# Abhipray/audio-codec

Hardware: AMD Instinct MI355X
Metric: audio channel-frames/s encode (48 kHz, 1024-line long blocks, 128 kb/s/ch) (higher is better)
Workload: dtype f64

## Files before the change

audio-codec_amd/csrc/k_psy.hip:

```cpp
#include "pacx_launch.h"
#include "mdct_dev.h"
#include "pcm_stage.h"
#include "wave_np_sum.h"
#include "quant_dev.h"


template <int DT>
__device__ __forceinline__ double hann_sample(const typename PcmStage<DT>::elem *raw, int i,
                                              const double *__restrict__ hw,
                                              const double *__restrict__ hw_pcm)
{
    if constexpr (DT == 0) {
        const int c = raw[i];
        return hw_pcm[i] * (double)(c == -32768 ? 0 : c);
    } else {
        return hw[i] * raw[i];
    }
}

#ifdef PACX_PSY_DEBUG
__device__ long long g_psy_dbg[16 * 16];
#define PSY_T(k) do { long long t_; asm volatile("s_waitcnt lgkmcnt(0)\n\ts_memtime %0\n\ts_waitcnt lgkmcnt(0)" : "=s"(t_) :: "memory"); \
                      if (dbg_on) dbg_acc[k] += t_ - dbg_last; dbg_last = t_; } while (0)
extern "C" int pacx_debug_read_psy(long long *out, int n)
// ... 591 lines not shown
#endif
#ifndef MASK_WG_PER_CU_PLAIN
#define MASK_WG_PER_CU_PLAIN 4
#endif



__device__ __forceinline__ unsigned long long mask_key_of(double v)
{
    const unsigned long long u = (unsigned long long)__double_as_longlong(v);
    return (u >> 63) ? ~u : (u | 0x8000000000000000ull);
}
__device__ __forceinline__ double mask_value_of(unsigned long long k)
{
    const unsigned long long u = (k >> 63) ? (k & 0x7fffffffffffffffull) : ~k;
    return __longlong_as_double((long long)u);
}

#ifndef MASK_WAVES_PLAIN
#define MASK_WAVES_PLAIN 4
#endif
constexpr int mask_waves(int m, bool tail) { return (m == PACX_M_LONG && !tail) ? MASK_WAVES_PLAIN : MASK_WAVES; }

template <int M, bool TAIL>
__global__ __launch_bounds__(64 * mask_waves(M, TAIL), (M == PACX_M_LONG && !TAIL) ? MASK_OCC_PLAIN : MASK_OCC) void k_mask(PacxTables T, const uint8_t *__restrict__ flags,
                                                         int n_ch, long long n_units, int mixed,
                                                         const PacxPeak *__restrict__ peaks,
                                                         const int32_t *__restrict__ n_peaks,
                                                         const double *__restrict__ lines,
                                                         double *__restrict__ smr,
                                                         double *__restrict__ thr_out,
                                                         const int32_t *__restrict__ cf_list,
                                                         const int32_t *__restrict__ cf_count,
                                                         MaskTail tail)
{
    constexpr bool SHORT = (M == PACX_M_SHORT);
    constexpr int NW = mask_waves(M, TAIL);
    static_assert(!(TAIL && SHORT), "the fused tail is for long blocks");
    constexpr int PER = M / 64;
    constexpr bool BARK_LDS = (MASK_LDS_TABLES & 1) != 0, QUIET_LDS = (MASK_LDS_TABLES & 2) != 0;
    __shared__ __attribute__((aligned(16))) double bark_l[BARK_LDS ? M : 1];
    __shared__ __attribute__((aligned(16))) double quiet_l[QUIET_LDS ? M : 1];
    __shared__ __attribute__((aligned(16))) double chunk_c[PER][4];
    constexpr bool PAD = M / 64 == 16;
    constexpr int RJ = PAD ? PER / 2 : 0;
    constexpr int NH = PAD ? 2 : 1, HP = PER / NH;
    constexpr int MH = M / NH;
    constexpr int JSTR = PAD ? 72 : 64;
    __shared__ __attribute__((aligned(16))) double bufs[NW][MH + (PAD ? MH / 8 : 0)];
    __shared__ __attribute__((aligned(16))) double2 mk_zs_all[NW][64];
    __shared__ __attribute__((aligned(16))) double mk_u_all[NW][64];
    const int tid = threadIdx.x, lane = tid & 63, wv = tid >> 6;
    const double *__restrict__ bark_g = SHORT ? T.bark_short : T.bark_long;
    const double *__restrict__ quiet_g = SHORT ? T.thresh_short : T.thresh_long;
    for (int i = tid; i < M; i += 64 * NW) {
        if (BARK_LDS)
            bark_l[i] = bark_g[i];
// ... 7 lines not shown
        double qm = quiet_s[64 * j + lane];
#pragma unroll
        for (int off = 32; off > 0; off >>= 1)
            qm = fmin(qm, __shfl_xor(qm, off, 64));
        if (lane == 0) {
            chunk_c[j][0] = bark_s[64 * j] - 0.5;
            chunk_c[j][1] = bark_s[64 * j + 63] + 0.5;
            chunk_c[j][2] = qm - 0.01;
        }
    }
    __syncthreads();

    double *buf = bufs[wv];
    const int sl = lane + (PAD ? lane >> 3 : 0);
    double2 *mk_zs = mk_zs_all[wv];
    double *mk_u = mk_u_all[wv];
    const int nb = SHORT ? T.nb_short : T.nb_long;
    const int32_t *__restrict__ lower = SHORT ? T.band_lower_short : T.band_lower_long;
    const int32_t *__restrict__ count = SHORT ? T.band_lines_short : T.band_lines_long;
    if (cf_list)
        n_units = SHORT ? (long long)(*cf_count) * PACX_SUB : (long long)(*cf_count);
#ifdef PACX_PSY_DEBUG
    const bool dbg_on = blockIdx.x == 5;
    long long dbg_acc[8] = {0, 0, 0, 0, 0, 0, 0, 0}, dbg_last = 0;
    unsigned long long st_pairs = 0, st_surv = 0, st_live = 0, st_batches = 0;
    PSY_T(7);
    dbg_acc[7] = 0;
#endif
    for (long long unit = (long long)blockIdx.x * NW + wv; unit < n_units;
         unit += (long long)gridDim.x * NW) {
        long long cf = SHORT ? unit / PACX_SUB : unit;
        const int sb = SHORT ? (int)(unit % PACX_SUB) : 0;
        if (cf_list) {
            cf = cf_list[cf];
        } else if (mixed) {
            const unsigned fl = flags ? flags[cf / n_ch] : 0u;
            if (SHORT != ((fl & 2u) != 0))
                continue;
        }
        const PacxPeak *__restrict__ pk = peaks + cf * PACX_MAX_PEAKS + sb * 64;
        const int np = n_peaks[cf * PACX_SUB + sb];
        const long long loff = cf * PACX_M_LONG + sb * PACX_M_SHORT;

        double rb[RJ ? RJ : 1];
#pragma unroll
        for (int j = 0; j < PER; ++j) {
            if (j < RJ)
// ... 73 lines not shown
                        pus[u] = mk_u[bs[u]];
                    }
#pragma unroll
                    for (int u = 0; u < 4; ++u) {
                        const double pz = zs[u].x, ps = zs[u].y, pu = pus[u];
                        const double dz = zj - pz;
                        const double a = fmax(fabs(dz) - 0.5, 0.0);
                        const double gain = (dz < 0.0 ? -27.0 : pu) * a;
                        const double cand = (ps + gain) - 16.0;
                        asm("v_max_f64 %0, %1, %2" : "=v"(bj) : "v"(bj), "v"(cand));
                    }
                }
                if (j < RJ)
                    rb[j] = bj;
                else
                    buf[sl + JSTR * (j - RJ)] = bj;
            }
        }
        wave_lds_fence();
        PSY_T(1);
        double *__restrict__ out = smr ? smr + cf * T.band_stride + sb * T.nb_short : nullptr;
        unsigned long long *key = (unsigned long long *)mk_zs;
        key[lane] = 0ull;
#pragma unroll 1
        for (int h = NH - 1; h >= 0; --h) {
            if (RJ && h == 0) {
                wave_lds_fence();
#pragma unroll
                for (int j = 0; j < RJ; ++j)
                    buf[sl + JSTR * j] = rb[j];
                wave_lds_fence();
            }
            const int k0 = h * MH;
            double v_next = lines[loff + k0 + lane], q_next = quiet_s[k0 + lane];
#pragma unroll 1
            for (int j = 0; j < HP; ++j) {
                const int k = k0 + lane + 64 * j;
                const double v = v_next;
                double thr = q_next;
                if (j + 1 < HP) {
                    v_next = lines[loff + k + 64];
                    q_next = quiet_s[k + 64];
                }
                const double bst = buf[sl + JSTR * j];
                if (bst > -INFINITY)
                    thr = fmax(thr, mask_round_trip(bst));
                if (thr_out)
                    thr_out[loff + k] = thr;
                double it = (v * v) * 4.0;
                if (it == 0.0)
                    it = 1e-8;
                double spl = 96.0 + 10.0 * pacx_log10_pos(it + PACX_EPS);
                if (spl < -30.0)
                    spl = -30.0;
                buf[sl + JSTR * j] = spl - thr;
            }
            wave_lds_fence();
            int rl = lane;
            asm volatile("" : "+v"(rl));
            double v[HP];
            uint8_t bd[HP];
            if constexpr (SHORT) {
                const double2 t = *(const double2 *)(buf + 2 * rl);
                v[0] = t.x;
                v[1] = t.y;
                const uchar2 b2 = *(const uchar2 *)(T.line_band_short + 2 * rl);
                bd[0] = b2.x;
                bd[1] = b2.y;
            } else {
                static_assert(SHORT || HP == 8, "eight lines per lane and half");
                const uint2 b8 = *(const uint2 *)(T.line_band_long + k0 + 8 * rl);
                const unsigned w[2] = {b8.x, b8.y};
#pragma unroll
                for (int j = 0; j < HP; ++j) {
                    v[j] = buf[9 * rl + j];
                    bd[j] = (uint8_t)(w[j >> 2] >> (8 * (j & 3)));
                }
            }
            wave_lds_fence();
            int cur = bd[0];
            double mx = v[0];
#pragma unroll
            for (int j = 1; j < HP; ++j) {
                if (bd[j] != cur) {
                    atomicMax(&key[cur], mask_key_of(mx));
                    cur = bd[j];
                    mx = v[j];
                } else {
                    mx = fmax(mx, v[j]);
                }
            }
            atomicMax(&key[cur], mask_key_of(mx));
        }
        wave_lds_fence();
        PSY_T(2);
        const double s_l = mask_value_of(key[lane & 31]);
        if (out && lane < nb)
            out[lane] = s_l;
        {
            if constexpr (TAIL) {
                wave_lds_fence();
                int tl = lane;
                asm volatile("" : "+v"(tl));
                char *base = (char *)buf;
                unsigned *words = (unsigned *)base;
                double *cp = (double *)(base + PACX_PAYLOAD_STRIDE);
                unsigned long long *bmax = (unsigned long long *)(base + 2704);
                int *ba_s = (int *)(base + 2960), *sf_s = ba_s + PACX_MAX_BANDS;
                int *offs = sf_s + PACX_MAX_BANDS, *lower_s = offs + PACX_MAX_BANDS + 1;
                const int half = tl >> 5, l = tl & 31;
                const unsigned fl = flags ? flags[cf / n_ch] : 0u;
                const long long boff = cf * T.band_stride;
                const int32_t *__restrict__ n_lines = T.use_sbr ? T.band_lines_long_alloc : T.band_lines_long;
                const double budget = pacx_bit_budget(T.target_bps, PACX_M_LONG, 0, (fl & 5u) != 0, T.n_scale_bits,
                                                      T.n_mant_size_bits, nb, T.use_vq, T.use_sbr);
// ... 72 lines not shown
                        if (tail.mantissa)
                            *(int4 *)(tail.mantissa + loff + k0 + j4) = make_int4(mq[0], mq[1], mq[2], mq[3]);
                    }
                    if (tail.status && __builtin_amdgcn_ballot_w64(near) && tl == 0)
                        atomicOr(&tail.status[cf], 16u);
                    if (tail.payload) {
                        wave_lds_fence();
                        const int nbytes = ((end - 3) + 4 + 7) >> 3;
                        unsigned *dst = (unsigned *)(tail.payload + cf * (long long)tail.payload_stride);
                        for (int i = tl; i < (nbytes + 3) / 4; i += 64)
                            dst[i] = __builtin_bswap32(words[i]);
                        if (tl == 0)
                            tail.n_bytes[cf] = nbytes;
                    }
                    PSY_T(6);
                }
            }
        }
        wave_lds_fence();
        PSY_T(3);
    }
#ifdef PACX_PSY_DEBUG
    if (dbg_on && lane == 0 && M == PACX_M_LONG)
        for (int k = 0; k < 8; ++k)
            g_psy_dbg[wv * 16 + k] = dbg_acc[k];
    if (lane == 0 && M == PACX_M_LONG) {
        atomicAdd((unsigned long long *)&g_psy_dbg[160], st_pairs);
        atomicAdd((unsigned long long *)&g_psy_dbg[161], st_surv);
        atomicAdd((unsigned long long *)&g_psy_dbg[162], st_live);
        atomicAdd((unsigned long long *)&g_psy_dbg[163], st_batches);
    }
#endif
}

#define SMRG_THREADS 256
__global__ __launch_bounds__(SMRG_THREADS) void k_smr_generic(long long n_blocks, int n, int nb,
                                                             const double *__restrict__ data,
                                                             const double *__restrict__ lines,
                                                             const double *__restrict__ hann,
                                                             const double *__restrict__ tw_cos,
                                                             const double *__restrict__ tw_sin, double norm,
                                                             double fstep, const double *__restrict__ bark,
                                                             const double *__restrict__ quiet,
                                                             const int32_t *__restrict__ band_lower,
                                                             const int32_t *__restrict__ band_count,
                                                             double *__restrict__ smr, double *__restrict__ thr_out,
                                                             int32_t *__restrict__ n_peaks_out)
{
    extern __shared__ __attribute__((aligned(16))) unsigned char smrg_lds[];
    const int half = n / 2, n_bins = half + 1, max_pk = half / 2 + 1;
    double *w = (double *)smrg_lds;
    double *inten = w + n;
    PacxPeak *pk = (PacxPeak *)(inten + n_bins + (n_bins & 1));
    __shared__ int n_pk;
    const int tid = threadIdx.x;
// ... 112 lines not shown
        launch_side<0, true>(T, in, flags, n_cf, short_blocks, mixed, peaks, n_peaks, n_kept, sbr_mean,
                             sbr_overall, st);
    else if (dtype == 0)
        launch_side<0, false>(T, in, flags, n_cf, short_blocks, mixed, peaks, n_peaks, n_kept, sbr_mean,
                              sbr_overall, st);
    else
        launch_side<1, false>(T, in, flags, n_cf, short_blocks, mixed, peaks, n_peaks, n_kept, sbr_mean,
                              sbr_overall, st);
}

void pacx_k::pacx_launch_front_long(const PacxTables &T, const PacxPcmView &in, long long n_cf, double *lines,
                                    int32_t *overall_scale, uint32_t *status, PacxPeak *peaks, int32_t *n_peaks,
                                    int32_t *n_kept, hipStream_t st)
{
    if (n_cf > 0)
        hipLaunchKernelGGL(k_front_long, dim3((unsigned)n_cf), dim3(64), 0, st, T, in, n_cf, lines, overall_scale,
                           status, peaks, n_peaks, n_kept);
}

void pacx_k::pacx_launch_mask(const PacxTables &T, const uint8_t *flags, int n_ch, long long n_cf,
                      int short_blocks, int mixed, const PacxPeak *peaks, const int32_t *n_peaks,
                      const double *lines, double *smr, double *thr_out, int n_cu,
                      const int32_t *list_long, const int32_t *list_short, const int32_t *counts,
                      const MaskTail *tail, hipStream_t st)
{
    if (n_cf <= 0)
        return;
    const int part = mixed >> 4;
    mixed &= 15;
    if ((!short_blocks || mixed) && part != 2) {
        const int nw = tail ? MASK_WAVES : MASK_WAVES_PLAIN;
        long long blocks = (n_cf + nw - 1) / nw;
        const long long per_cu = tail ? MASK_WG_PER_CU : MASK_WG_PER_CU_PLAIN;
        if (blocks > per_cu * n_cu)
            blocks = per_cu * n_cu;
        if (tail)
            hipLaunchKernelGGL((k_mask<PACX_M_LONG, true>), dim3((unsigned)blocks), dim3(64 * MASK_WAVES), 0, st, T,
                               flags, n_ch, n_cf, mixed, peaks, n_peaks, lines, (double *)nullptr, thr_out,
                               mixed ? list_long : nullptr, counts, *tail);
        else
            hipLaunchKernelGGL((k_mask<PACX_M_LONG, false>), dim3((unsigned)blocks), dim3(64 * MASK_WAVES_PLAIN), 0, st, T,
                               flags, n_ch, n_cf, mixed, peaks, n_peaks, lines, smr, thr_out,
                               mixed ? list_long : nullptr, counts, MaskTail{});
    }
    if ((short_blocks || mixed) && part != 1) {
        const long long units = n_cf * PACX_SUB;
        long long blocks = (units + MASK_WAVES - 1) / MASK_WAVES;
        if (blocks > (32LL / MASK_WAVES) * n_cu)
            blocks = (32LL / MASK_WAVES) * n_cu;
        hipLaunchKernelGGL((k_mask<PACX_M_SHORT, false>), dim3((unsigned)blocks), dim3(64 * MASK_WAVES), 0, st, T,
                           flags, n_ch, units, mixed, peaks, n_peaks, lines, smr, thr_out,
                           mixed ? list_short : nullptr, counts ? counts + 1 : nullptr, MaskTail{});
    }
}
```

audio-codec_amd/csrc/pacx_api.hip:

```cpp
#include <hip/hip_runtime.h>

#include <math.h>
#include <stdio.h>
#include <stdlib.h>
#include <string.h>

#include <cmath>
#include <string>
#include <vector>

#include "../../include/pacx.h"
#include "body_index.h"
#include "pacx_launch.h"
#include "pvq_dev.h"
#include "pacx_vq_tables.h"
#include "pacx_tables_gen.h"

using namespace pacx_k;

struct PacxOverrides {
    int split_short;
    int fuse_tail;
    int fuse_front;
    int vq_fuse_alloc;
    int vq_frame;
    int vq_bfs;
    int vq_dec_frame;
};

#define PACX_FUSE_FRONT_DEFAULT 1

static int env_override(const char *name, int lo, int hi)
{
    const char *e = getenv(name);
    if (!e || !*e)
        return -1;
    char *end;
    const long v = strtol(e, &end, 10);
    return (*end || v < lo || v > hi) ? -1 : (int)v;
}

static PacxOverrides read_overrides(void)
{
    PacxOverrides o;
    o.split_short = env_override("PACX_SPLIT_SHORT", 0, 0);
    o.fuse_tail = env_override("PACX_FUSE_TAIL", 0, 1);
    o.fuse_front = env_override("PACX_FUSE_FRONT", 0, 1);
    o.vq_fuse_alloc = env_override("PACX_VQ_FUSE_ALLOC", 0, 1);
    o.vq_frame = env_override("PACX_VQ_FRAME", 0, 0);
    o.vq_bfs = env_override("PACX_VQ_BFS", 0, 1 << 20);
    o.vq_dec_frame = env_override("PACX_VQ_DEC_FRAME", 0, 0);
    return o;
}

struct pacx_handle {
    int device;
    int n_cu;
    PacxOverrides force;
    PacxTables T;
    std::vector<void *> owned;
    long long ws_cf;
    double *ws_lines;
    double *ws_smr;
    PacxPeak *ws_peaks;
    int32_t *ws_npeaks;
    int32_t *ws_nkept;
    int32_t *ws_overall;
    long long *ws_chunks;
    long long *ws_offs;
    int32_t *ws_lists;
// ... 12 lines not shown
    int32_t *ws_mant;
    long long ws_dec_cf;
    double *ws_dec_lines;
    uint8_t *ws_dec_sbr;
    uint32_t *ws_dec_status;
    double *ws_sbr_mean;
    long long ws_vq_cf;
    unsigned *ws_unit_words;
    int32_t *ws_unit_bits;
    long long ws_index_bytes;
    char *ws_index;
    long long ws_thr_cf;
    double *ws_thr;
    uint32_t *ws_rate_status;
    long long ws_solve_n;
    char *ws_solve;
    long long *ws_seg;
    long long seg_host_n;
    long long *seg_host;
    hipEvent_t ev_seg;
    std::string err;
};

static thread_local std::string g_create_err;

static int fail(pacx_handle *h, int code, const std::string &msg)
{
    if (h)
        h->err = msg;
    else
        g_create_err = msg;
    return code;
}

#define HIP_TRY(h, call)                                                               \
    do {                                                                               \
        hipError_t e_ = (call);                                                        \
        if (e_ != hipSuccess)                                                          \
            return fail(h, PACX_E_HIP, std::string(#call) + ": " + hipGetErrorString(e_)); \
    } while (0)

static void drain_internal(pacx_handle *h);
#define HIP_TRY_FORKED(h, call)                                                        \
    do {                                                                               \
        hipError_t e_ = (call);                                                        \
        if (e_ != hipSuccess) {                                                        \
// ... 655 lines not shown
extern "C" int pacx_smr_batch(pacx_handle *h, const pacx_pcm *in, const double *lines, int short_blocks,
                              double *smr, double *threshold, int32_t *n_peaks, void *stream)
{
    if (!h)
        return PACX_E_ARG;
    PacxPcmView v;
    int fast;
    long long n_cf;
    int rc = check_pcm(h, in, &v, &fast, &n_cf);
    if (rc)
        return rc;
    if (n_cf == 0)
        return PACX_OK;
    if (!lines || !smr)
        return fail(h, PACX_E_ARG, "pacx_smr_batch: lines or smr is null");
    HIP_TRY(h, hipSetDevice(h->device));
    if ((rc = pacx_reserve(h, n_cf)))
        return rc;
    hipStream_t st = (hipStream_t)stream;
    const int sb = short_blocks ? 1 : 0;
    pacx_launch_side(h->T, v, in->dtype, fast, nullptr, n_cf, sb, 0, h->ws_peaks, h->ws_npeaks, h->ws_nkept,
                     nullptr, nullptr, st);
    pacx_launch_mask(h->T, nullptr, in->n_channels, n_cf, sb, 0, h->ws_peaks, h->ws_nkept, lines, smr,
                     threshold, h->n_cu, nullptr, nullptr, nullptr, nullptr, st);
    if (n_peaks) {
        if (sb)
            HIP_TRY(h, hipMemcpyAsync(n_peaks, h->ws_npeaks, (size_t)n_cf * PACX_SUB * sizeof(int32_t),
                                      hipMemcpyDeviceToDevice, st));
        else
            HIP_TRY(h, hipMemcpy2DAsync(n_peaks, sizeof(int32_t), h->ws_npeaks, PACX_SUB * sizeof(int32_t),
                                        sizeof(int32_t), (size_t)n_cf, hipMemcpyDeviceToDevice, st));
    }
    return post_launch(h, "pacx_smr_batch");
}

extern "C" int pacx_smr_generic_batch(pacx_handle *h, int64_t n_blocks, int n_samples, const double *data,
                                      const double *lines, const pacx_smr_tables *t, double *smr, double *threshold,
                                      int32_t *n_peaks, void *stream)
{
    if (!h)
        return PACX_E_ARG;
    if (n_blocks == 0)
        return PACX_OK;
    if (n_blocks < 0 || !data || !lines || !smr || !t || !t->hann || !t->tw_cos || !t->tw_sin || !t->bark ||
        !t->quiet || !t->band_lower || !t->band_lines)
        return fail(h, PACX_E_ARG, "pacx_smr_generic_batch: bad argument");
    if (n_samples < 16 || n_samples > 8192 || (n_samples & 1) || t->n_bands < 1 || t->n_bands > PACX_MAX_BANDS)
// ... 76 lines not shown
    {
        if (fast) {
            mdct_long(st);
            if (mixed)
                mdct_short(st);
        } else {
            pacx_launch_mdct(h->T, v, dtype, fast, frame_flags, n_cf, 0, mixed, 0, h->ws_lines, overall_scale, PACX_SUB,
                             status, st);
        }
    }
    void side(int part, bool sbr, hipStream_t st) const
    {
        pacx_launch_side(h->T, v, dtype, fast, frame_flags, n_cf, 0, mixed | part, h->ws_peaks, h->ws_npeaks, h->ws_nkept,
                         sbr ? h->ws_sbr_mean : nullptr, sbr ? overall_scale : nullptr, st);
    }
    void front_long(hipStream_t st) const
    {
        pacx_launch_front_long(h->T, v, n_cf, h->ws_lines, overall_scale, status, h->ws_peaks, h->ws_npeaks,
                               h->ws_nkept, st);
    }
    void mask(int part, const MaskTail *tail, hipStream_t st) const
    {
        pacx_launch_mask(h->T, frame_flags, n_ch, n_cf, 0, mixed | part, h->ws_peaks, h->ws_nkept, h->ws_lines, h->ws_smr,
                         nullptr, h->n_cu, list_long, list_short, counts, tail, st);
    }
};

static int encode_scalar(pacx_handle *h, const pacx_pcm *in, const uint8_t *frame_flags,
                         int32_t *overall_scale, int32_t *scale_factor, int32_t *bit_alloc,
                         int32_t *mantissa, uint32_t *status, uint8_t *payload, int32_t *n_bytes,
                         void *stream, const char *what)
{
    if (!h)
        return PACX_E_ARG;
    PacxPcmView v;
    int fast;
    long long n_cf;
    int rc = check_pcm(h, in, &v, &fast, &n_cf);
    if (rc)
        return rc;
    if (n_cf == 0)
        return PACX_OK;
    if (!overall_scale || !scale_factor || !bit_alloc || !status || (!payload && !mantissa) ||
        (payload && !n_bytes))
        return fail(h, PACX_E_ARG, std::string(what) + ": null output pointer");
    if (h->T.use_vq)
        return fail(h, PACX_E_UNSUPPORTED, std::string(what) + ": handle was created with use_vq "
// ... 580 lines not shown
{
    if (!h)
        return PACX_E_ARG;
    PacxPcmView v;
    int fast;
    long long n_cf;
    int rc = check_pcm(h, in, &v, &fast, &n_cf);
    if (rc)
        return rc;
    if (n_cf == 0)
        return PACX_OK;
    if (!dec_lines || !overall_scale || !noise || !mask || !nmr_db)
        return fail(h, PACX_E_ARG, "pacx_nmr_batch: null pointer");
    HIP_TRY(h, hipSetDevice(h->device));
    if ((rc = pacx_reserve(h, n_cf)) || (rc = grow(h, GROW_NMR, n_cf)))
        return rc;
    hipStream_t st = (hipStream_t)stream;
    const EncodeStep s(h, in, v, fast, frame_flags, n_cf, h->ws_overall, nullptr);
    if (s.mixed)
        s.lists(st);
    s.mdct(st);
    s.side(0, false, st);
    pacx_launch_mask(h->T, frame_flags, s.n_ch, n_cf, 0, s.mixed, h->ws_peaks, h->ws_nkept, h->ws_lines, h->ws_smr,
                     h->ws_thr, h->n_cu, s.list_long, s.list_short, s.counts, nullptr, st);
    pacx_launch_nmr(h->T, frame_flags, s.n_ch, n_cf, h->ws_lines, dec_lines, overall_scale, h->ws_thr, status, noise, mask,
                    nmr_db, st);
    return post_launch(h, "pacx_nmr_batch");
}

enum { BUDGET_SEARCH, BUDGET_GIVEN, ALLOC_GIVEN };
static int encode_budgeted(pacx_handle *h, const pacx_pcm *in, const uint8_t *frame_flags, int mode,
                           double target_nmr_db, double max_bits_per_sample, const int32_t *budget_in,
                           const int32_t *alloc_in, int32_t *overall_scale, int32_t *scale_factor, int32_t *bit_alloc, int32_t *mantissa,
                           uint32_t *status, uint8_t *payload, int32_t *n_bytes, int32_t *budget_out, void *stream,
                           const char *what)
{
    if (!h)
        return PACX_E_ARG;
    if (h->T.use_vq || h->T.use_sbr)
        return fail(h, PACX_E_UNSUPPORTED, std::string(what) + ": scalar handles only (created without use_vq, use_sbr)");
    const bool search = mode == BUDGET_SEARCH, given = mode == ALLOC_GIVEN;
    if (search && !std::isfinite(target_nmr_db))
        return fail(h, PACX_E_ARG, std::string(what) + ": target_nmr_db is not finite");
    if (search && !(max_bits_per_sample > 0.0 && max_bits_per_sample <= 16.0))
        return fail(h, PACX_E_ARG, std::string(what) + ": max_bits_per_sample must lie in (0, 16]");
    PacxPcmView v;
    int fast;
// ... 6 lines not shown
        return fail(h, PACX_E_ARG, std::string(what) + ": null pointer");
    if (n_cf == 0)
        return PACX_OK;
    HIP_TRY(h, hipSetDevice(h->device));
    if ((rc = pacx_reserve(h, n_cf)) || (search && (rc = grow(h, GROW_NMR, n_cf))))
        return rc;
    if (!mantissa) {
        if ((rc = grow(h, GROW_MANT, n_cf)))
            return rc;
        mantissa = h->ws_mant;
    }
    hipStream_t st = (hipStream_t)stream;
    if (!fast) {
        HIP_TRY(h, hipMemsetAsync(status, 0, (size_t)n_cf * sizeof(uint32_t), st));
        HIP_TRY(h, hipMemsetAsync(overall_scale, 0, (size_t)n_cf * PACX_SUB * sizeof(int32_t), st));
    }
    const EncodeStep s(h, in, v, fast, frame_flags, n_cf, overall_scale, status);
    if (s.mixed)
        s.lists(st);
    s.mdct(st);
    if (!given) {
        s.side(0, false, st);
        pacx_launch_mask(h->T, frame_flags, s.n_ch, n_cf, 0, s.mixed, h->ws_peaks, h->ws_nkept, h->ws_lines, h->ws_smr,
                         search ? h->ws_thr : nullptr, h->n_cu, s.list_long, s.list_short, s.counts, nullptr, st);
    }
    if (given)
        pacx_launch_band_sanitize(h->T, frame_flags, s.n_ch, n_cf, alloc_in, bit_alloc, status, PACX_PAYLOAD_STRIDE, st);
    else if (search)
        pacx_launch_rate_search(h->T, frame_flags, s.n_ch, n_cf, target_nmr_db, max_bits_per_sample, h->ws_lines,
                                h->ws_thr, h->ws_smr, overall_scale, budget_out, bit_alloc, status, st);
    else
        pacx_launch_bitalloc_budget(h->T, frame_flags, s.n_ch, n_cf, budget_in, h->ws_smr, bit_alloc, status, st);
    pacx_launch_quantize(h->T, frame_flags, s.n_ch, n_cf, 0, s.mixed, h->ws_lines, overall_scale, PACX_SUB, bit_alloc,
                         scale_factor, mantissa, st);
    pacx_launch_pack(h->T, frame_flags, s.n_ch, n_cf, overall_scale, scale_factor, bit_alloc, mantissa, status, payload,
                     PACX_PAYLOAD_STRIDE, n_bytes, st);
    return post_launch(h, what);
}

extern "C" int pacx_encode_pack_nmr_batch(pacx_handle *h, const pacx_pcm *in, const uint8_t *frame_flags,
                                          double target_nmr_db, double max_bits_per_sample, int32_t *overall_scale,
                                          int32_t *scale_factor, int32_t *bit_alloc, int32_t *mantissa, uint32_t *status,
                                          uint8_t *payload, int32_t *n_bytes, int32_t *budget, void *stream)
{
    return encode_budgeted(h, in, frame_flags, BUDGET_SEARCH, target_nmr_db, max_bits_per_sample, nullptr, nullptr, overall_scale,
                           scale_factor, bit_alloc, mantissa, status, payload, n_bytes, budget, stream,
                           "pacx_encode_pack_nmr_batch");
// ... 66 lines not shown
    if (!worst || !bits || !steps)
        return fail(h, PACX_E_ARG, std::string(what) + ": null pointer");
    int need, sub_stride;
    rate_curve_layout(h->T, max_bits_per_sample, &need, &sub_stride);
    if (row < need)
        return fail(h, PACX_E_ARG, std::string(what) + ": row is smaller than pacx_rate_curve_layout's (" +
                                       std::to_string(need) + ")");
    if (n_cf == 0)
        return PACX_OK;
    HIP_TRY(h, hipSetDevice(h->device));
    if ((rc = pacx_reserve(h, n_cf)) || (rc = grow(h, GROW_NMR, n_cf)))
        return rc;
    hipStream_t st = (hipStream_t)stream;
    if (!fast) {
        HIP_TRY(h, hipMemsetAsync(h->ws_rate_status, 0, (size_t)n_cf * sizeof(uint32_t), st));
        HIP_TRY(h, hipMemsetAsync(h->ws_overall, 0, (size_t)n_cf * PACX_SUB * sizeof(int32_t), st));
    }
    const EncodeStep s(h, in, v, fast, frame_flags, n_cf, h->ws_overall, h->ws_rate_status);
    if (s.mixed)
        s.lists(st);
    s.mdct(st);
    s.side(0, false, st);
    pacx_launch_mask(h->T, frame_flags, s.n_ch, n_cf, 0, s.mixed, h->ws_peaks, h->ws_nkept, h->ws_lines, h->ws_smr,
                     h->ws_thr, h->n_cu, s.list_long, s.list_short, s.counts, nullptr, st);
    pacx_launch_rate_curve(h->T, frame_flags, s.n_ch, n_cf, max_bits_per_sample, row, sub_stride, h->ws_lines, h->ws_thr,
                           h->ws_smr, h->ws_overall, h->ws_rate_status, worst, bits, steps, st);
    return post_launch(h, what);
}

static int solve_range(pacx_handle *h, const char *what, double nmr_lo_db, double nmr_hi_db, int *t_lo, int *t_hi)
{
    const double bound = 1048576.0;
    if (!std::isfinite(nmr_lo_db) || !std::isfinite(nmr_hi_db) || fabs(nmr_lo_db) > bound || fabs(nmr_hi_db) > bound)
        return fail(h, PACX_E_ARG, std::string(what) + ": target bounds must be finite (at most 2^20 dB in magnitude)");
    const double lo64 = nmr_lo_db * PACX_RATE_TARGET_GRID, hi64 = nmr_hi_db * PACX_RATE_TARGET_GRID;
    if (lo64 != floor(lo64) || hi64 != floor(hi64))
        return fail(h, PACX_E_ARG, std::string(what) + ": target bounds must be multiples of 1/64 dB");
    if (lo64 > hi64)
        return fail(h, PACX_E_ARG, std::string(what) + ": nmr_lo_db is above nmr_hi_db");
    *t_lo = (int)lo64;
    *t_hi = (int)hi64;
    return PACX_OK;
}

static int check_segments(pacx_handle *h, const char *what, int64_t n_cf, int64_t n_seg, const int64_t *seg_first,
                          const int64_t *limit_bytes)
{
// ... 133 lines not shown
    int rc = check_pcm(h, in, &v, &fast, &n_cf);
    if (rc)
        return rc;
    if (!nmr || !cap || !cap_alloc)
        return fail(h, PACX_E_ARG, std::string(what) + ": null pointer");
    if (band_record_bound(h->T, max_bits_per_sample) > PACX_PAYLOAD_STRIDE)
        return fail(h, PACX_E_UNSUPPORTED, std::string(what) + ": a record at this cap rate would not fit pacx_payload_stride");
    if (n_cf == 0)
        return PACX_OK;
    HIP_TRY(h, hipSetDevice(h->device));
    if ((rc = pacx_reserve(h, n_cf)) || (rc = grow(h, GROW_NMR, n_cf)))
        return rc;
    hipStream_t st = (hipStream_t)stream;
    if (!fast) {
        HIP_TRY(h, hipMemsetAsync(h->ws_rate_status, 0, (size_t)n_cf * sizeof(uint32_t), st));
        HIP_TRY(h, hipMemsetAsync(h->ws_overall, 0, (size_t)n_cf * PACX_SUB * sizeof(int32_t), st));
    }
    const EncodeStep s(h, in, v, fast, frame_flags, n_cf, h->ws_overall, h->ws_rate_status);
    if (s.mixed)
        s.lists(st);
    s.mdct(st);
    s.side(0, false, st);
    pacx_launch_mask(h->T, frame_flags, s.n_ch, n_cf, 0, s.mixed, h->ws_peaks, h->ws_nkept, h->ws_lines, h->ws_smr,
                     h->ws_thr, h->n_cu, s.list_long, s.list_short, s.counts, nullptr, st);
    pacx_launch_band_curve(h->T, frame_flags, s.n_ch, n_cf, max_bits_per_sample, h->ws_lines, h->ws_thr, h->ws_smr,
                           h->ws_overall, h->ws_rate_status, nmr, cap, cap_alloc, st);
    return post_launch(h, what);
}

extern "C" int pacx_band_pick(pacx_handle *h, int64_t n_cf, const double *nmr, const int32_t *cap, const int32_t *cap_alloc,
                              double target_nmr_db, int32_t *bit_alloc, int32_t *n_bytes, uint8_t *capped, void *stream)
{
    const char *what = "pacx_band_pick";
    if (!h)
        return PACX_E_ARG;
    if (h->T.use_vq || h->T.use_sbr)
        return fail(h, PACX_E_UNSUPPORTED, std::string(what) + ": scalar handles only (created without use_vq, use_sbr)");
    if (n_cf < 0 || n_cf > 0x7fffffffLL / PACX_SUB)
        return fail(h, PACX_E_ARG, std::string(what) + ": bad channel-frame count");
    if (n_cf > 0 && (!nmr || !cap || !cap_alloc || !bit_alloc || !n_bytes || !capped))
        return fail(h, PACX_E_ARG, std::string(what) + ": null pointer");
    if (!std::isfinite(target_nmr_db))
        return fail(h, PACX_E_ARG, std::string(what) + ": target_nmr_db is not finite");
    HIP_TRY(h, hipSetDevice(h->device));
    pacx_launch_band_pick(h->T, n_cf, target_nmr_db, nmr, cap, cap_alloc, bit_alloc, n_bytes, capped, (hipStream_t)stream);
    return post_launch(h, what);
}
// ... 71 lines not shown
```

audio-codec_amd/csrc/pacx_exact.h:

```cpp
#ifndef PACX_EXACT_H
#define PACX_EXACT_H

#include <math.h>
#include <stdint.h>
#include <string.h>

#if defined(__HIPCC__)
#define PACX_HD __host__ __device__ __forceinline__
#else
#define PACX_HD static inline
#endif

#define PACX_MAX_BANDS 32
#define PACX_ALLOC_MAX_PASSES 200
#define PACX_DB_PER_BIT 6.2
#define PACX_EPS 2.220446049250313e-16
#define PACX_VQ_SPLIT_BITS 32
#define PACX_VQ_THETA_TABLE_BITS 12

PACX_HD double pacx_pcm16_to_f64(int c)
{
    const int neg = c < 0;
    const int mag = (neg ? -c : c) & 32767;
    const double n = (double)(2 * mag);
// ... 419 lines not shown
    PACX_FMA_SC(p, f, p, c4);
    PACX_FMA_SC(p, f, p, c3);
    PACX_FMA_SC(p, f, p, c2);
    PACX_FMA_SC(p, f, p, c1);
#undef PACX_FMA_SC
    p = fma(f, p, 1.0);
    int e = (int)n;
    return ldexp(p, e);
}

PACX_HD double pacx_spl_of_intensity_of(double x)
{
    double y = (96.0 - x) * 0.33219280948873623;
    if (y > 1000.0)
        y = 1000.0;
    const double t = PACX_EPS * pacx_exp2_lean(y);
    if (!(t < 1e-3))
        return -30.0;
    const double p = t * (1.0 + t * (-0.5 + t * (1.0 / 3.0 + t * (-0.25 + t * 0.2))));
    const double r = x + 4.3429448190325182765 * p;
    return r < -30.0 ? -30.0 : r;
}

PACX_HD double pacx_spl_scalar(double intensity)
{
    if (intensity == 0.0)
        return -30.0;
    double spl = 96.0 + 10.0 * log10(fabs(intensity) + PACX_EPS);
    if (spl < -30.0)
        spl = -30.0;
    return spl;
}

PACX_HD double pacx_bark(double f)
{
    const double t = f / 7500.0;
    return 13.0 * atan(0.76 * f / 1000.0) + 3.5 * atan(t * t);
}

PACX_HD double pacx_thresh_quiet(double f)
{
    if (f < 10.0)
        f = 10.0;
    const double k = f / 1000.0;
    const double d = k - 3.3;
    return 3.64 * pow(k, -0.8) - 6.5 * exp(-0.6 * (d * d)) + 0.001 * (k * k * k * k);
// ... 14 lines not shown
```

audio-codec_amd/csrc/pacx_launch.h:

```cpp
#ifndef PACX_LAUNCH_H
#define PACX_LAUNCH_H

#include "../../include/pacx.h"
#include "pacx_dev.h"

struct PvqTables;

namespace pacx_k {

void pacx_launch_mdct(const PacxTables &T, const PacxPcmView &in, int dtype, int fast,
                      const uint8_t *flags, long long n_cf, int short_blocks, int mixed, int prewin,
                      double *lines, int32_t *scale_out, int scale_stride, uint32_t *status,
                      hipStream_t st);
void pacx_launch_mdct_v2(const PacxTables &T, const PacxPcmView &in, const uint8_t *flags, long long n_cf,
                         int skip_cur, double *lines, int32_t *scale_out, int scale_stride,
                         uint32_t *status_init, int n_cu, const int32_t *cf_list, const int32_t *cf_count,
                         hipStream_t st);
void pacx_launch_mdct_x2(const PacxTables &T, const PacxPcmView &in, long long n_cf, double *lines,
                         int32_t *scale_out, int scale_stride, uint32_t *status_init, int n_cu, hipStream_t st);

void pacx_launch_side(const PacxTables &T, const PacxPcmView &in, int dtype, int fast,
                      const uint8_t *flags, long long n_cf, int short_blocks, int mixed,
                      PacxPeak *peaks, int32_t *n_peaks, int32_t *n_kept, double *sbr_mean,
                      int32_t *sbr_overall, hipStream_t st);
void pacx_launch_front_long(const PacxTables &T, const PacxPcmView &in, long long n_cf, double *lines,
                            int32_t *overall_scale, uint32_t *status, PacxPeak *peaks, int32_t *n_peaks,
                            int32_t *n_kept, hipStream_t st);
void pacx_launch_mask(const PacxTables &T, const uint8_t *flags, int n_ch, long long n_cf,
                      int short_blocks, int mixed, const PacxPeak *peaks, const int32_t *n_peaks,
                      const double *lines, double *smr, double *thr_out, int n_cu,
                      const int32_t *list_long, const int32_t *list_short, const int32_t *counts,
                      const MaskTail *tail, hipStream_t st);
size_t pacx_smr_generic_lds(int n);
void pacx_launch_smr_generic(long long n_blocks, int n, int nb, const double *data, const double *lines,
                             const double *hann, const double *tw_cos, const double *tw_sin, double norm, double fstep,
                             const double *bark, const double *quiet, const int32_t *band_lower,
                             const int32_t *band_count, double *smr, double *thr_out, int32_t *n_peaks_out,
                             hipStream_t st);

void pacx_launch_bitalloc(const PacxTables &T, const uint8_t *flags, int n_ch, long long n_cf,
                          int short_blocks, int mixed, int skip_long, const double *smr, int32_t *bit_alloc,
                          uint32_t *status, hipStream_t st);
void pacx_launch_quantize(const PacxTables &T, const uint8_t *flags, int n_ch, long long n_cf,
                          int short_blocks, int mixed, const double *lines, const int32_t *overall,
                          int overall_stride, const int32_t *bit_alloc, int32_t *scale_factor,
                          int32_t *mantissa, hipStream_t st);
void pacx_launch_pack(const PacxTables &T, const uint8_t *flags, int n_ch, long long n_cf,
                      const int32_t *overall, const int32_t *scale_factor, const int32_t *bit_alloc,
                      const int32_t *mantissa, const uint32_t *status, uint8_t *payload,
                      int payload_stride, int32_t *n_bytes, hipStream_t st);
void pacx_launch_tail(const PacxTables &T, const uint8_t *flags, int n_ch, long long n_cf, const double *smr,
                      const double *lines, const int32_t *overall, int32_t *bit_alloc, int32_t *scale_factor,
                      int32_t *mantissa, uint32_t *status, uint8_t *payload, int payload_stride,
                      int32_t *n_bytes, const int32_t *list_short, const int32_t *count_short, int skip_long,
                      hipStream_t st);
// ... 119 lines not shown
```

Measured before the change: 52.29 million.

## Screen long-block mask lines with float bounds before exact f64 SMR computation

For long blocks without a threshold output, each line's SPL-minus-threshold is first bounded cheaply in float using a hardware log2. Per-band maxima of the lower bounds are gathered with LDS atomics, and only lines whose upper bound can reach the band maximum go through the exact double-precision log and round-trip path. Candidates are compacted via ballot/mbcnt into an LDS list. This aims to cut the f64 log10 and mask round-trip work per line, but adds a compaction pass and relies on the error margins being conservative enough to keep exact results.

```diff
diff --git a/audio-codec_amd/csrc/k_psy.hip b/audio-codec_amd/csrc/k_psy.hip
--- a/audio-codec_amd/csrc/k_psy.hip
+++ b/audio-codec_amd/csrc/k_psy.hip
@@ -637,17 +637,34 @@
 #endif
 constexpr int mask_waves(int m, bool tail) { return (m == PACX_M_LONG && !tail) ? MASK_WAVES_PLAIN : MASK_WAVES; }
 
-template <int M, bool TAIL>
-__global__ __launch_bounds__(64 * mask_waves(M, TAIL), (M == PACX_M_LONG && !TAIL) ? MASK_OCC_PLAIN : MASK_OCC) void k_mask(PacxTables T, const uint8_t *__restrict__ flags,
-                                                         int n_ch, long long n_units, int mixed,
-                                                         const PacxPeak *__restrict__ peaks,
-                                                         const int32_t *__restrict__ n_peaks,
-                                                         const double *__restrict__ lines,
-                                                         double *__restrict__ smr,
-                                                         double *__restrict__ thr_out,
-                                                         const int32_t *__restrict__ cf_list,
-                                                         const int32_t *__restrict__ cf_count,
-                                                         MaskTail tail)
+__device__ __forceinline__ int mask_fkey_of(int bits) { return bits ^ ((bits >> 31) & 0x7fffffff); }
+
+#define MASK_LIST 256
+
+__device__ __forceinline__ double mask_line_exact(double v, double bst, double &thr)
+{
+    if (bst > -INFINITY)
+        thr = fmax(thr, mask_round_trip(bst));
+    double it = (v * v) * 4.0;
+    if (it == 0.0)
+        it = 1e-8;
+    double spl = 96.0 + 10.0 * pacx_log10_pos(it + PACX_EPS);
+    if (spl < -30.0)
+        spl = -30.0;
+    return spl - thr;
+}
+
+template <int M, bool TAIL, bool SCREEN>
+__device__ __forceinline__ void mask_body(const PacxTables &T, const uint8_t *__restrict__ flags,
+                                          int n_ch, long long n_units, int mixed,
+                                          const PacxPeak *__restrict__ peaks,
+                                          const int32_t *__restrict__ n_peaks,
+                                          const double *__restrict__ lines,
+                                          double *__restrict__ smr,
+                                          double *__restrict__ thr_out,
+                                          const int32_t *__restrict__ cf_list,
+                                          const int32_t *__restrict__ cf_count,
+                                          const MaskTail &tail)
 {
     constexpr bool SHORT = (M == PACX_M_SHORT);
     constexpr int NW = mask_waves(M, TAIL);
@@ -701,7 +718,7 @@
         n_units = SHORT ? (long long)(*cf_count) * PACX_SUB : (long long)(*cf_count);
 #ifdef PACX_PSY_DEBUG
     const bool dbg_on = blockIdx.x == 5;
-    long long dbg_acc[8] = {0, 0, 0, 0, 0, 0, 0, 0}, dbg_last = 0;
+    long long dbg_acc[10] = {0, 0, 0, 0, 0, 0, 0, 0, 0, 0}, dbg_last = 0;
     unsigned long long st_pairs = 0, st_surv = 0, st_live = 0, st_batches = 0;
     PSY_T(7);
     dbg_acc[7] = 0;
@@ -821,75 +838,158 @@
         double *__restrict__ out = smr ? smr + cf * T.band_stride + sb * T.nb_short : nullptr;
         unsigned long long *key = (unsigned long long *)mk_zs;
         key[lane] = 0ull;
+        if constexpr (SCREEN) {
+            int *fkey = (int *)(mk_zs + 32);
+            unsigned short *list = (unsigned short *)mk_u;
+            static_assert(!SCREEN || (PAD && HP == 8), "long blocks: eight lines per lane and half, padded halves");
+            const uint8_t *__restrict__ line_band = T.line_band_long;
+            constexpr int LSTR = HP + 1;
 #pragma unroll 1
-        for (int h = NH - 1; h >= 0; --h) {
-            if (RJ && h == 0) {
+            for (int h = NH - 1; h >= 0; --h) {
+                if (RJ && h == 0) {
+                    wave_lds_fence();
+#pragma unroll
+                    for (int j = 0; j < RJ; ++j)
+                        buf[sl + JSTR * j] = rb[j];
+                }
+                const int k0 = h * MH;
+                fkey[lane] = (int)0x80000000;
                 wave_lds_fence();
-#pragma unroll
-                for (int j = 0; j < RJ; ++j)
-                    buf[sl + JSTR * j] = rb[j];
+                int rl = lane;
+                asm volatile("" : "+v"(rl));
+                float d_lo[HP], d_hi[HP];
+                uint8_t bd[HP];
+                {
+                    const uint2 b8 = *(const uint2 *)(T.line_band_long + k0 + 8 * rl);
+                    const unsigned w[2] = {b8.x, b8.y};
+#pragma unroll
+                    for (int j = 0; j < HP; ++j)
+                        bd[j] = (uint8_t)(w[j >> 2] >> (8 * (j & 3)));
+                }
+                {
+                    const double2 *__restrict__ lp = (const double2 *)(lines + loff + k0 + HP * rl);
+                    const double2 *__restrict__ qp = (const double2 *)(quiet_s + k0 + HP * rl);
+#pragma unroll
+                    for (int j = 0; j < HP; j += 2) {
+                        const double2 v2 = lp[j >> 1], q2 = qp[j >> 1];
+                        pacx_mask_bound(v2.x, buf[LSTR * rl + j], q2.x, &d_lo[j], &d_hi[j]);
+                        pacx_mask_bound(v2.y, buf[LSTR * rl + j + 1], q2.y, &d_lo[j + 1], &d_hi[j + 1]);
+                    }
+                }
+                {
+                    int cur = bd[0];
+                    float mx = d_lo[0];
+#pragma unroll
+                    for (int j = 1; j < HP; ++j) {
+                        if (bd[j] != cur) {
+                            atomicMax(&fkey[cur], mask_fkey_of(__float_as_int(mx)));
+                            cur = bd[j];
+                            mx = d_lo[j];
+                        } else {
+                            mx = fmaxf(mx, d_lo[j]);
+                        }
+                    }
+                    atomicMax(&fkey[cur], mask_fkey_of(__float_as_int(mx)));
+                }
                 wave_lds_fence();
+                fkey[lane] = mask_fkey_of(fkey[lane]);
+                wave_lds_fence();
+                unsigned cm = 0;
+#pragma unroll
+                for (int j = 0; j < HP; ++j)
+                    cm |= (d_hi[j] >= __int_as_float(fkey[bd[j]])) ? 1u << j : 0u;
+                PSY_T(8);
+                int base = 0, total;
+#pragma unroll 1
+                do {
+                    int run = 0;
+#pragma unroll
+                    for (int j = 0; j < HP; ++j) {
+                        const bool c = (cm >> j) & 1u;
+                        const unsigned long long m = __builtin_amdgcn_ballot_w64(c);
+                        const int pos = run - base + (int)__builtin_amdgcn_mbcnt_hi((unsigned)(m >> 32),
+                                                         __builtin_amdgcn_mbcnt_lo((unsigned)m, 0u));
+                        if (c && (unsigned)pos < (unsigned)MASK_LIST)
+                            list[pos] = (unsigned short)(HP * rl + j);
+                        run += __popcll(m);
+                    }
+                    total = run;
+                    wave_lds_fence();
+                    const int n = min(MASK_LIST, total - base);
+                    for (int i = lane; i < n; i += 64) {
+                        const int kk = list[i], k = k0 + kk;
+                        double thr = quiet_s[k];
+                        const double d = mask_line_exact(lines[loff + k], buf[kk + (kk >> 3)], thr);
+                        atomicMax(&key[line_band[k]], mask_key_of(d));
+                    }
+                    wave_lds_fence();
+                    base += MASK_LIST;
+                } while (base < total);
+                PSY_T(9);
             }
-            const int k0 = h * MH;
-            double v_next = lines[loff + k0 + lane], q_next = quiet_s[k0 + lane];
+        } else {
 #pragma unroll 1
-            for (int j = 0; j < HP; ++j) {
-                const int k = k0 + lane + 64 * j;
-                const double v = v_next;
-                double thr = q_next;
-                if (j + 1 < HP) {
-                    v_next = lines[loff + k + 64];
-                    q_next = quiet_s[k + 64];
+            for (int h = NH - 1; h >= 0; --h) {
+                if (RJ && h == 0) {
+                    wave_lds_fence();
+#pragma unroll
+                    for (int j = 0; j < RJ; ++j)
+                        buf[sl + JSTR * j] = rb[j];
+                    wave_lds_fence();
                 }
-                const double bst = buf[sl + JSTR * j];
-                if (bst > -INFINITY)
-                    thr = fmax(thr, mask_round_trip(bst));
-                if (thr_out)
-                    thr_out[loff + k] = thr;
-                double it = (v * v) * 4.0;
-                if (it == 0.0)
-                    it = 1e-8;
-                double spl = 96.0 + 10.0 * pacx_log10_pos(it + PACX_EPS);
-                if (spl < -30.0)
-                    spl = -30.0;
-                buf[sl + JSTR * j] = spl - thr;
+                const int k0 = h * MH;
+                double v_next = lines[loff + k0 + lane], q_next = quiet_s[k0 + lane];
+#pragma unroll 1
+                for (int j = 0; j < HP; ++j) {
+                    const int k = k0 + lane + 64 * j;
+                    const double v = v_next;
+                    double thr = q_next;
+                    if (j + 1 < HP) {
+                        v_next = lines[loff + k + 64];
+                        q_next = quiet_s[k + 64];
+                    }
+                    const double d = mask_line_exact(v, buf[sl + JSTR * j], thr);
+                    if (thr_out)
+                        thr_out[loff + k] = thr;
+                    buf[sl + JSTR * j] = d;
+                }
+                wave_lds_fence();
+                int rl = lane;
+                asm volatile("" : "+v"(rl));
+                double v[HP];
+                uint8_t bd[HP];
+                if constexpr (SHORT) {
+                    const double2 t = *(const double2 *)(buf + 2 * rl);
+                    v[0] = t.x;
+                    v[1] = t.y;
+                    const uchar2 b2 = *(const uchar2 *)(T.line_band_short + 2 * rl);
+                    bd[0] = b2.x;
+                    bd[1] = b2.y;
+                } else {
+                    static_assert(SHORT || HP == 8, "eight lines per lane and half");
+                    const uint2 b8 = *(const uint2 *)(T.line_band_long + k0 + 8 * rl);
+                    const unsigned w[2] = {b8.x, b8.y};
+#pragma unroll
+                    for (int j = 0; j < HP; ++j) {
+                        v[j] = buf[9 * rl + j];
+                        bd[j] = (uint8_t)(w[j >> 2] >> (8 * (j & 3)));
+                    }
+                }
+                wave_lds_fence();
+                int cur = bd[0];
+                double mx = v[0];
+#pragma unroll
+                for (int j = 1; j < HP; ++j) {
+                    if (bd[j] != cur) {
+                        atomicMax(&key[cur], mask_key_of(mx));
+                        cur = bd[j];
+                        mx = v[j];
+                    } else {
+                        mx = fmax(mx, v[j]);
+                    }
+                }
+                atomicMax(&key[cur], mask_key_of(mx));
             }
-            wave_lds_fence();
-            int rl = lane;
-            asm volatile("" : "+v"(rl));
-            double v[HP];
-            uint8_t bd[HP];
-            if constexpr (SHORT) {
-                const double2 t = *(const double2 *)(buf + 2 * rl);
-                v[0] = t.x;
-                v[1] = t.y;
-                const uchar2 b2 = *(const uchar2 *)(T.line_band_short + 2 * rl);
-                bd[0] = b2.x;
-                bd[1] = b2.y;
-            } else {
-                static_assert(SHORT || HP == 8, "eight lines per lane and half");
-                const uint2 b8 = *(const uint2 *)(T.line_band_long + k0 + 8 * rl);
-                const unsigned w[2] = {b8.x, b8.y};
-#pragma unroll
-                for (int j = 0; j < HP; ++j) {
-                    v[j] = buf[9 * rl + j];
-                    bd[j] = (uint8_t)(w[j >> 2] >> (8 * (j & 3)));
-                }
-            }
-            wave_lds_fence();
-            int cur = bd[0];
-            double mx = v[0];
-#pragma unroll
-            for (int j = 1; j < HP; ++j) {
-                if (bd[j] != cur) {
-                    atomicMax(&key[cur], mask_key_of(mx));
-                    cur = bd[j];
-                    mx = v[j];
-                } else {
-                    mx = fmax(mx, v[j]);
-                }
-            }
-            atomicMax(&key[cur], mask_key_of(mx));
         }
         wave_lds_fence();
         PSY_T(2);
@@ -1008,7 +1108,7 @@
     }
 #ifdef PACX_PSY_DEBUG
     if (dbg_on && lane == 0 && M == PACX_M_LONG)
-        for (int k = 0; k < 8; ++k)
+        for (int k = 0; k < 10; ++k)
             g_psy_dbg[wv * 16 + k] = dbg_acc[k];
     if (lane == 0 && M == PACX_M_LONG) {
         atomicAdd((unsigned long long *)&g_psy_dbg[160], st_pairs);
@@ -1017,6 +1117,26 @@
         atomicAdd((unsigned long long *)&g_psy_dbg[163], st_batches);
     }
 #endif
+}
+
+#define MASK_KERNEL_ARGS PacxTables T, const uint8_t *__restrict__ flags, int n_ch, long long n_units, int mixed, \
+                         const PacxPeak *__restrict__ peaks, const int32_t *__restrict__ n_peaks, \
+                         const double *__restrict__ lines, double *__restrict__ smr, double *__restrict__ thr_out, \
+                         const int32_t *__restrict__ cf_list, const int32_t *__restrict__ cf_count, MaskTail tail
+#define MASK_BOUNDS(M, TAIL) __launch_bounds__(64 * mask_waves(M, TAIL), (M == PACX_M_LONG && !TAIL) ? MASK_OCC_PLAIN : MASK_OCC)
+
+template <int M, bool TAIL>
+__global__ MASK_BOUNDS(M, TAIL) void k_mask(MASK_KERNEL_ARGS)
+{
+    mask_body<M, TAIL, M == PACX_M_LONG>(T, flags, n_ch, n_units, mixed, peaks, n_peaks, lines, smr,
+                                         M == PACX_M_LONG ? nullptr : thr_out, cf_list, cf_count, tail);
+}
+
+template <int M, bool TAIL>
+__global__ MASK_BOUNDS(M, TAIL) void k_mask_full(MASK_KERNEL_ARGS)
+{
+    mask_body<M, TAIL, false>(T, flags, n_ch, n_units, mixed, peaks, n_peaks, lines, smr, thr_out, cf_list, cf_count,
+                              tail);
 }
 
 #define SMRG_THREADS 256
@@ -1175,7 +1295,7 @@
                       int short_blocks, int mixed, const PacxPeak *peaks, const int32_t *n_peaks,
                       const double *lines, double *smr, double *thr_out, int n_cu,
                       const int32_t *list_long, const int32_t *list_short, const int32_t *counts,
-                      const MaskTail *tail, hipStream_t st)
+                      const MaskTail *tail, int screen, hipStream_t st)
 {
     if (n_cf <= 0)
         return;
@@ -1187,12 +1307,15 @@
         const long long per_cu = tail ? MASK_WG_PER_CU : MASK_WG_PER_CU_PLAIN;
         if (blocks > per_cu * n_cu)
             blocks = per_cu * n_cu;
+        const bool full = thr_out || !screen;
+        auto *const k_tail = full ? k_mask_full<PACX_M_LONG, true> : k_mask<PACX_M_LONG, true>;
+        auto *const k_plain = full ? k_mask_full<PACX_M_LONG, false> : k_mask<PACX_M_LONG, false>;
         if (tail)
-            hipLaunchKernelGGL((k_mask<PACX_M_LONG, true>), dim3((unsigned)blocks), dim3(64 * MASK_WAVES), 0, st, T,
+            hipLaunchKernelGGL(k_tail, dim3((unsigned)blocks), dim3(64 * MASK_WAVES), 0, st, T,
                                flags, n_ch, n_cf, mixed, peaks, n_peaks, lines, (double *)nullptr, thr_out,
                                mixed ? list_long : nullptr, counts, *tail);
         else
-            hipLaunchKernelGGL((k_mask<PACX_M_LONG, false>), dim3((unsigned)blocks), dim3(64 * MASK_WAVES_PLAIN), 0, st, T,
+            hipLaunchKernelGGL(k_plain, dim3((unsigned)blocks), dim3(64 * MASK_WAVES_PLAIN), 0, st, T,
                                flags, n_ch, n_cf, mixed, peaks, n_peaks, lines, smr, thr_out,
                                mixed ? list_long : nullptr, counts, MaskTail{});
     }
diff --git a/audio-codec_amd/csrc/pacx_api.hip b/audio-codec_amd/csrc/pacx_api.hip
--- a/audio-codec_amd/csrc/pacx_api.hip
+++ b/audio-codec_amd/csrc/pacx_api.hip
@@ -22,6 +22,7 @@
     int split_short;
     int fuse_tail;
     int fuse_front;
+    int mask_screen;
     int vq_fuse_alloc;
     int vq_frame;
     int vq_bfs;
@@ -29,6 +30,7 @@
 };
 
 #define PACX_FUSE_FRONT_DEFAULT 1
+#define PACX_MASK_SCREEN_DEFAULT 1
 
 static int env_override(const char *name, int lo, int hi)
 {
@@ -46,6 +48,7 @@
     o.split_short = env_override("PACX_SPLIT_SHORT", 0, 0);
     o.fuse_tail = env_override("PACX_FUSE_TAIL", 0, 1);
     o.fuse_front = env_override("PACX_FUSE_FRONT", 0, 1);
+    o.mask_screen = env_override("PACX_MASK_SCREEN", 0, 1);
     o.vq_fuse_alloc = env_override("PACX_VQ_FUSE_ALLOC", 0, 1);
     o.vq_frame = env_override("PACX_VQ_FRAME", 0, 0);
     o.vq_bfs = env_override("PACX_VQ_BFS", 0, 1 << 20);
@@ -104,6 +107,11 @@
     std::string err;
 };
 
+static int mask_screen(const pacx_handle *h)
+{
+    return h->force.mask_screen >= 0 ? h->force.mask_screen : PACX_MASK_SCREEN_DEFAULT;
+}
+
 static thread_local std::string g_create_err;
 
 static int fail(pacx_handle *h, int code, const std::string &msg)
@@ -805,7 +813,7 @@
     pacx_launch_side(h->T, v, in->dtype, fast, nullptr, n_cf, sb, 0, h->ws_peaks, h->ws_npeaks, h->ws_nkept,
                      nullptr, nullptr, st);
     pacx_launch_mask(h->T, nullptr, in->n_channels, n_cf, sb, 0, h->ws_peaks, h->ws_nkept, lines, smr,
-                     threshold, h->n_cu, nullptr, nullptr, nullptr, nullptr, st);
+                     threshold, h->n_cu, nullptr, nullptr, nullptr, nullptr, mask_screen(h), st);
     if (n_peaks) {
         if (sb)
             HIP_TRY(h, hipMemcpyAsync(n_peaks, h->ws_npeaks, (size_t)n_cf * PACX_SUB * sizeof(int32_t),
@@ -928,7 +936,7 @@
     void mask(int part, const MaskTail *tail, hipStream_t st) const
     {
         pacx_launch_mask(h->T, frame_flags, n_ch, n_cf, 0, mixed | part, h->ws_peaks, h->ws_nkept, h->ws_lines, h->ws_smr,
-                         nullptr, h->n_cu, list_long, list_short, counts, tail, st);
+                         nullptr, h->n_cu, list_long, list_short, counts, tail, mask_screen(h), st);
     }
 };
 
@@ -1555,7 +1563,7 @@
     s.mdct(st);
     s.side(0, false, st);
     pacx_launch_mask(h->T, frame_flags, s.n_ch, n_cf, 0, s.mixed, h->ws_peaks, h->ws_nkept, h->ws_lines, h->ws_smr,
-                     h->ws_thr, h->n_cu, s.list_long, s.list_short, s.counts, nullptr, st);
+                     h->ws_thr, h->n_cu, s.list_long, s.list_short, s.counts, nullptr, mask_screen(h), st);
     pacx_launch_nmr(h->T, frame_flags, s.n_ch, n_cf, h->ws_lines, dec_lines, overall_scale, h->ws_thr, status, noise, mask,
                     nmr_db, st);
     return post_launch(h, "pacx_nmr_batch");
@@ -1608,7 +1616,7 @@
     if (!given) {
         s.side(0, false, st);
         pacx_launch_mask(h->T, frame_flags, s.n_ch, n_cf, 0, s.mixed, h->ws_peaks, h->ws_nkept, h->ws_lines, h->ws_smr,
-                         search ? h->ws_thr : nullptr, h->n_cu, s.list_long, s.list_short, s.counts, nullptr, st);
+                         search ? h->ws_thr : nullptr, h->n_cu, s.list_long, s.list_short, s.counts, nullptr, mask_screen(h), st);
     }
     if (given)
         pacx_launch_band_sanitize(h->T, frame_flags, s.n_ch, n_cf, alloc_in, bit_alloc, status, PACX_PAYLOAD_STRIDE, st);
@@ -1721,7 +1729,7 @@
     s.mdct(st);
     s.side(0, false, st);
     pacx_launch_mask(h->T, frame_flags, s.n_ch, n_cf, 0, s.mixed, h->ws_peaks, h->ws_nkept, h->ws_lines, h->ws_smr,
-                     h->ws_thr, h->n_cu, s.list_long, s.list_short, s.counts, nullptr, st);
+                     h->ws_thr, h->n_cu, s.list_long, s.list_short, s.counts, nullptr, mask_screen(h), st);
     pacx_launch_rate_curve(h->T, frame_flags, s.n_ch, n_cf, max_bits_per_sample, row, sub_stride, h->ws_lines, h->ws_thr,
                            h->ws_smr, h->ws_overall, h->ws_rate_status, worst, bits, steps, st);
     return post_launch(h, what);
@@ -1901,7 +1909,7 @@
     s.mdct(st);
     s.side(0, false, st);
     pacx_launch_mask(h->T, frame_flags, s.n_ch, n_cf, 0, s.mixed, h->ws_peaks, h->ws_nkept, h->ws_lines, h->ws_smr,
-                     h->ws_thr, h->n_cu, s.list_long, s.list_short, s.counts, nullptr, st);
+                     h->ws_thr, h->n_cu, s.list_long, s.list_short, s.counts, nullptr, mask_screen(h), st);
     pacx_launch_band_curve(h->T, frame_flags, s.n_ch, n_cf, max_bits_per_sample, h->ws_lines, h->ws_thr, h->ws_smr,
                            h->ws_overall, h->ws_rate_status, nmr, cap, cap_alloc, st);
     return post_launch(h, what);
diff --git a/audio-codec_amd/csrc/pacx_exact.h b/audio-codec_amd/csrc/pacx_exact.h
--- a/audio-codec_amd/csrc/pacx_exact.h
+++ b/audio-codec_amd/csrc/pacx_exact.h
@@ -465,6 +465,37 @@
     return r < -30.0 ? -30.0 : r;
 }
 
+#define PACX_MASK_RT_SPAN 4.4e-3f
+#define PACX_MASK_BOUND_ERR 2e-3f
+#define PACX_MASK_SPL_CAP 481.0f
+
+PACX_HD float pacx_mask_bound_arg(double v)
+{
+    double it = (v * v) * 4.0;
+    if (it == 0.0)
+        it = 1e-8;
+    return (float)(it + PACX_EPS);
+}
+
+PACX_HD void pacx_mask_bound_of(float l2, double bst, double quiet, float *d_lo, float *d_hi)
+{
+    const float spl = fmaxf(fmaf(l2, 3.01029995663981195f, 96.0f), -30.0f);
+    const float m = fmaxf((float)quiet, (float)bst);
+    *d_hi = (spl - m) + PACX_MASK_BOUND_ERR;
+    *d_lo = (fminf(spl, PACX_MASK_SPL_CAP) - fmaxf(m, -30.0f)) - (PACX_MASK_RT_SPAN + PACX_MASK_BOUND_ERR);
+}
+
+PACX_HD void pacx_mask_bound(double v, double bst, double quiet, float *d_lo, float *d_hi)
+{
+    const float a = pacx_mask_bound_arg(v);
+#if defined(__HIP_DEVICE_COMPILE__)
+    const float l2 = __builtin_amdgcn_logf(a);
+#else
+    const float l2 = log2f(a);
+#endif
+    pacx_mask_bound_of(l2, bst, quiet, d_lo, d_hi);
+}
+
 PACX_HD double pacx_spl_scalar(double intensity)
 {
     if (intensity == 0.0)
diff --git a/audio-codec_amd/csrc/pacx_launch.h b/audio-codec_amd/csrc/pacx_launch.h
--- a/audio-codec_amd/csrc/pacx_launch.h
+++ b/audio-codec_amd/csrc/pacx_launch.h
@@ -30,7 +30,7 @@
                       int short_blocks, int mixed, const PacxPeak *peaks, const int32_t *n_peaks,
                       const double *lines, double *smr, double *thr_out, int n_cu,
                       const int32_t *list_long, const int32_t *list_short, const int32_t *counts,
-                      const MaskTail *tail, hipStream_t st);
+                      const MaskTail *tail, int screen, hipStream_t st);
 size_t pacx_smr_generic_lds(int n);
 void pacx_launch_smr_generic(long long n_blocks, int n, int nb, const double *data, const double *lines,
                              const double *hann, const double *tw_cos, const double *tw_sin, double norm, double fstep,
```

After: 56.12 million (median of 6 runs). 1.07x the previous value.
